# js0n-lai/my-nope-nerf

Measured on AMD Instinct MI355X. Metric: training rays/sec at 1024 rays×128 samples; PSNR parity (±0.1 dB) vs ref, higher is better.
Workload: dtype f32 (f16x3 emulation); 1 GPU; config 2: V_KITTI scene-1 shape 188x621, 1024 rays x 128 samples per GPU, poses fixed, full train_step (render fwd+bwd, rgb-l2+depth-l1, Adam); global_batch=1024, seq_len=128, hidden_dim=256, parallelism=dp1

## Files before the change

my-nope-nerf_amd/csrc/field_bwd.cpp:

```cpp
#include "common.hpp"

#include <cstdlib>
#include <vector>

namespace {

constexpr int L = NERF_BWD_LAYERS;
constexpr int D = 256, HR = 128;
constexpr int OUT_P[L] = {D, D, D, D, D, D, D, D, D, HR};
constexpr int K1[L] = {64, D, D, D, D, D, D, D, D, D};
constexpr int KP[L] = {64, D, D, D, D + 64, D, D, D, D, D + 64};
constexpr int SEG[L] = {0, 0, 0, 0, 1, 0, 0, 0, 0, 2};
constexpr int NREF[L] = {D, D, D, D, D, D, D, D, D, HR};
constexpr int KREF[L] = {63, D, D, D, D + 63, D, D, D, D, D + 27};
constexpr int LF = 8, LR = 9;

struct Carve {
    char* base;
    size_t off = 0;
    float* take(size_t n) {
        off = (off + 255) & ~size_t(255);
        float* p = base ? reinterpret_cast<float*>(base + off) : nullptr;
        off += n * sizeof(float);
        return p;
    }
};

struct Work {
    float *graw4, *dyr, *dyr_rm, *dyr_cm, *part, *hpart, *scratch;
    float *dx[L], *dx_rm[L], *dx_cm[L];
    float *genc_p0, *genc_p4, *genc_d;
    float *slab[L], *bslab[L];
    int splits[L];
};

size_t carve(char* base, int np, int ray_grad, Work& w) {
    Carve c{base};
    w.graw4 = c.take((size_t)np * 4);
    w.dyr = c.take((size_t)np * HR);
    w.dyr_rm = c.take(np);
    w.dyr_cm = c.take((size_t)(np / 128) * HR);
    w.part = c.take((size_t)nerf_heads_part_size(D, np));
    w.hpart = c.take((size_t)nerf::heads_part_blocks(np) * (256 + 384 + 4));
    w.scratch = c.take(512);
    for (int l = 1; l < L; ++l) {
        w.dx[l] = c.take((size_t)np * K1[l]);
        w.dx_rm[l] = c.take(np);
        w.dx_cm[l] = c.take((size_t)(np / 128) * K1[l]);
    }
    w.dx[0] = w.dx_rm[0] = w.dx_cm[0] = nullptr;
    w.genc_p0 = ray_grad ? c.take((size_t)np * 64) : nullptr;
    w.genc_p4 = ray_grad ? c.take((size_t)np * 64) : nullptr;
    w.genc_d = ray_grad ? c.take((size_t)np * 64) : nullptr;
    for (int l = 0; l < L; ++l) w.splits[l] = nerf_linear_bwd_weight_splits(OUT_P[l], K1[l], np);
    for (int l = 0; l < L; ++l) {
        w.slab[l] = c.take((size_t)w.splits[l] * OUT_P[l] * KP[l]);
        w.bslab[l] = c.take((size_t)w.splits[l] * OUT_P[l]);
    }
    return c.off + 256;
}

struct EventPool {
    std::vector<hipEvent_t> ev;
    size_t next = 0;
    hipEvent_t get() {
        if (next == ev.size()) {
            hipEvent_t e;
            if (hipEventCreateWithFlags(&e, hipEventDisableTiming) != hipSuccess) return nullptr;
            ev.push_back(e);
        }
        return ev[next++];
    }
};
thread_local EventPool g_events;

#define RC(x)                \
    do {                     \
        const int rc_ = (x); \
        if (rc_) return rc_; \
    } while (0)

int fork(hipStream_t main, hipStream_t side) {
    hipEvent_t e = g_events.get();
    NERF_CHECK(e != nullptr, "nerf_field_backward: hipEventCreate failed");
    NERF_CHECK(hipEventRecord(e, main) == hipSuccess && hipStreamWaitEvent(side, e, 0) == hipSuccess,
// ... 23 lines not shown
    hipStream_t main = nerf::as_stream(stream), side = nerf::as_stream(side_stream);
    nerf_chain_bwd c{};
    c.graw4 = graw4;
    c.hr_mask = a.mask[LR];
    c.ld_hr_mask = HR / 32;
    c.wd = a.wd;
    c.wc = a.wc;
    for (int i = 0; i < 9; ++i) {
        const int l = LR - i;
        c.wt_img[i] = a.wt_cimg[l];
        c.wt_img_rows[i] = KP[l];
        c.in_mask[i] = l == LR ? nullptr : a.mask[l - 1];
        c.ld_in_mask[i] = OUT_P[l - 1 < 0 ? 0 : l - 1] / 32;
    }
    c.dy[0] = w.dyr; c.lddy[0] = HR; c.dy_cmax[0] = w.dyr_cm; c.dy_rmax[0] = w.dyr_rm;
    for (int i = 1; i < 10; ++i) {
        const int l = 10 - i;
        c.dy[i] = w.dx[l]; c.lddy[i] = K1[l]; c.dy_cmax[i] = w.dx_cm[l]; c.dy_rmax[i] = w.dx_rm[l];
    }
    c.scratch = w.scratch;
    c.n_pad = np;
    RC(nerf_mlp_chain_bwd(&c, stream));
    if (heads_after) {
        RC(nerf_heads_bwd_mode(2, graw4, a.act[7], D, a.act[LR], HR, nullptr, 0, D, a.wc, nullptr, 0, w.part, np,
                               nullptr, nullptr, stream));
        RC(nerf_heads_reduce(w.part, D, np, a.g_wd, a.g_bd, a.g_wc, a.g_bc, 0, stream));
    }
    auto dy_of = [&](int l, const float*& dy, const float*& cm, const float*& rm) {
        if (l == LR) { dy = w.dyr; cm = w.dyr_cm; rm = w.dyr_rm; }
        else { dy = w.dx[l + 1]; cm = w.dx_cm[l + 1]; rm = w.dx_rm[l + 1]; }
    };
    const char* ws = std::getenv("NERF_WGRAD_SCHED");
    const int sched = ws ? std::atoi(ws) : 3;
    if (sched == 3) {
        nerf::SlabJobDesc jobs[nerf::kSlabJobsMax];
        int nj = 0;
        for (int e = 0; e < n_extra; ++e) jobs[nj++] = extra[e];
        auto flush = [&](hipStream_t s) -> int {
            if (s != main) RC(fork(main, s));
            RC(nerf::slab_reduce_jobs(jobs, nj, s));
            nj = 0;
            return NERF_OK;
        };
        auto job = [&](int l) {
            jobs[nj++] = nerf::SlabJobDesc{w.slab[l], w.splits[l], OUT_P[l], KP[l], NREF[l], KREF[l], w.bslab[l], a.gw[l],
                                           a.gb[l]};
        };
        auto enc_rows = [&](int l) -> int {
            if (!a.ray_grad) return NERF_OK;
            const float *dy, *cm, *rm;
            dy_of(l, dy, cm, rm);
            const int op = OUT_P[l];
            const int k0 = l == 0 ? 0 : K1[l];
            float* out = l == LR ? w.genc_d : l == 4 ? w.genc_p4 : w.genc_p0;
            return nerf_linear_bwd_data(dy, op, op, a.wt[l] + (size_t)k0 * op, a.wt_img[l] + (size_t)k0 * 8, KP[l], nullptr,
                                        0, nullptr, nullptr, 0, out, 64, np, 64, rm, nullptr, nullptr, stream);
        };
        nerf_wgrad_tile_job tj[nerf::kWgradJobsMax];
        int tgrp[nerf::kWgradJobsMax];
        int nt = 0, cur_grp = 0;
        auto tiles = [&](int l) {
            const float *dy, *cm, *rm;
            dy_of(l, dy, cm, rm);
            const int op = OUT_P[l];
            const float* x = l == 0 ? a.enc_p : a.act[l - 1];
            const float* xcm = l == 0 ? a.enc_p_cmax : a.cmax[l - 1];
            tgrp[nt] = cur_grp;
            tj[nt++] = nerf_wgrad_tile_job{dy, op, op, x, K1[l], K1[l], w.splits[l], w.slab[l], KP[l], 0, w.bslab[l], cm, xcm};
            if (SEG[l]) {
                tgrp[nt] = cur_grp;
                tj[nt++] = nerf_wgrad_tile_job{dy, op, op, SEG[l] == 1 ? a.enc_p : a.enc_d, 64, 64, w.splits[l], w.slab[l],
                                               KP[l], K1[l], nullptr, cm, SEG[l] == 1 ? a.enc_p_cmax : a.enc_d_cmax};
            }
            job(l);
        };
        auto launch = [&]() -> int {
            RC(nerf_linear_bwd_weight_jobs(tj, nt, np, w.splits[LF], stream));
            nt = 0;
            return NERF_OK;
        };
        const char* wgg = std::getenv("NERF_WGRAD_GROUPS");
        const int groups = w.splits[LF] % 16 == 0 ? (wgg ? std::atoi(wgg) : 2) : 0;
        const int s2 = w.splits[LF] / 2;
        if (groups >= 2) {
            for (int l : {LF, 7, 6, 5}) w.splits[l] = s2;
            w.splits[LR] = 2 * s2;
            tiles(LR);
            tgrp[nt - 1] = 1;
            for (int l : {LF, 7}) tiles(l);
            cur_grp = 1;
            for (int l : {6, 5}) tiles(l);
            cur_grp = 0;
            RC(nerf_linear_bwd_weight_job_groups(tj, tgrp, nt, np, s2, 2, stream));
            nt = 0;
        } else {
            for (int l : {LR, LF, 7, 6, 5}) tiles(l);
            RC(launch());
        }
        const char* b1 = std::getenv("NERF_WGRAD_BATCH1");
        const int batch1 = b1 ? std::atoi(b1) : 2;
        if (batch1 != 2) RC(flush(batch1 == 0 ? side : main));
        RC(enc_rows(LR));
        if (groups >= 1) {
            for (int l : {1, 2, 3, 4}) w.splits[l] = s2;
            w.splits[0] = 2 * s2;
            tiles(4);
            tgrp[nt - 1] = 1;
            for (int l : {3, 0}) tiles(l);
            cur_grp = 1;
            for (int l : {2, 1}) tiles(l);
            cur_grp = 0;
            RC(nerf_linear_bwd_weight_job_groups(tj, tgrp, nt, np, s2, 2, stream));
            nt = 0;
        } else {
            for (int l : {3, 2, 1, 4, 0}) tiles(l);
            RC(launch());
        }
        RC(flush(main));
        RC(enc_rows(4));
        RC(enc_rows(0));
    } else if (sched == 2) {
        nerf::SlabJobDesc jobs[nerf::kSlabJobsMax];
        int nj = 0;
        for (int e = 0; e < n_extra; ++e) jobs[nj++] = extra[e];
        auto flush = [&](hipStream_t s) -> int {
            if (s != main) RC(fork(main, s));
            RC(nerf::slab_reduce_jobs(jobs, nj, s));
            nj = 0;
            return NERF_OK;
        };
        auto job = [&](int l) {
            jobs[nj++] = nerf::SlabJobDesc{w.slab[l], w.splits[l], OUT_P[l], KP[l], NREF[l], KREF[l], w.bslab[l], a.gw[l],
                                           a.gb[l]};
        };
        auto enc_rows = [&](int l) -> int {
            if (!a.ray_grad) return NERF_OK;
            const float *dy, *cm, *rm;
            dy_of(l, dy, cm, rm);
            const int op = OUT_P[l];
            const int k0 = l == 0 ? 0 : K1[l];
            float* out = l == LR ? w.genc_d : l == 4 ? w.genc_p4 : w.genc_p0;
            return nerf_linear_bwd_data(dy, op, op, a.wt[l] + (size_t)k0 * op, a.wt_img[l] + (size_t)k0 * 8, KP[l], nullptr,
                                        0, nullptr, nullptr, 0, out, 64, np, 64, rm, nullptr, nullptr, stream);
        };
        {
            const float *dy, *cm, *rm;
            dy_of(LR, dy, cm, rm);
            RC(nerf_linear_bwd_weight(dy, HR, HR, a.act[LF], K1[LR], K1[LR], np, w.splits[LR], w.slab[LR], KP[LR], 0,
                                      w.bslab[LR], cm, a.cmax[LF], stream));
            RC(nerf_linear_bwd_weight(dy, HR, HR, a.enc_d, 64, 64, np, w.splits[LR], w.slab[LR], KP[LR], K1[LR], nullptr,
                                      cm, a.enc_d_cmax, stream));
            job(LR);
            RC(enc_rows(LR));
        }
        {
            nerf_wgrad_job wj[nerf::kWgradPairsMax];
            int n = 0;
            for (int l = LF; l >= 1; --l) {
                const float *dy, *cm, *rm;
                dy_of(l, dy, cm, rm);
                NERF_CHECK(OUT_P[l] == D && K1[l] == D && w.splits[l] == w.splits[LF], "layer %d", l);
                wj[n++] = nerf_wgrad_job{dy, D, a.act[l - 1], D, w.slab[l], KP[l], w.bslab[l], cm, a.cmax[l - 1]};
                if (l != 4) job(l);
            }
            RC(nerf_linear_bwd_weight_multi(wj, n, np, w.splits[LF], stream));
        }
        RC(flush(side));
        {
            const float *dy4, *cm4, *rm4, *dy0, *cm0, *rm0;
            dy_of(4, dy4, cm4, rm4);
            dy_of(0, dy0, cm0, rm0);
            RC(nerf::wgrad_narrow_pair(dy4, D, a.enc_p, 64, w.splits[4], w.slab[4], KP[4], K1[4], nullptr, cm4, a.enc_p_cmax,
                                       dy0, D, a.enc_p, 64, w.splits[0], w.slab[0], KP[0], 0, w.bslab[0], cm0, a.enc_p_cmax,
                                       np, main));
            job(4);
            job(0);
            RC(enc_rows(4));
            RC(enc_rows(0));
        }
        RC(flush(main));
    } else {
        nerf::SlabJobDesc jobs[nerf::kSlabJobsMax];
        int nj = 0;
        for (int e = 0; e < n_extra; ++e) jobs[nj++] = extra[e];
        auto flush = [&](hipStream_t s) -> int {
            if (s != main) RC(fork(main, s));
            RC(nerf::slab_reduce_jobs(jobs, nj, s));
            nj = 0;
            return NERF_OK;
        };
// ... 278 lines not shown
```

my-nope-nerf_amd/csrc/gemm.hpp:

```cpp
#pragma once
#include "common.hpp"

namespace nerf {

typedef float f32x16 __attribute__((ext_vector_type(16)));

__device__ __forceinline__ int acc_row(int r, int hi) { return (r & 3) + 8 * (r >> 2) + 4 * hi; }

template <int TM, int TN>
__device__ __forceinline__ void zero_acc(f32x16 (&acc)[TM][TN]) {
#pragma unroll
    for (int i = 0; i < TM; ++i)
#pragma unroll
        for (int j = 0; j < TN; ++j)
#pragma unroll
            for (int r = 0; r < 16; ++r) acc[i][j][r] = 0.f;
}

struct NTArgs {
    const float* a1; int lda1; int k1;
    const float* a2; int lda2; int k2;
    const float* b;  int ldb;
    const uint16_t* bs; int bs_rows;
    const float* bias;
// ... 456 lines not shown
            }
        }
    }
    if (HD && nh) {
#pragma unroll
        for (int i = 0; i < TM; ++i)
#pragma unroll
            for (int c = 0; c < 3; ++c)
                if (c < nh) {
                    const float v = hp[c][i] + __shfl_xor(hp[c][i], 32, 64);
                    if (hf == 0) lhs[(wm0 + 32 * i + sl) * 3 + c] = v;
                }
    }
    if constexpr (H) {
#pragma unroll
        for (int i = 0; i < TM; ++i) {
            const float m = fmaxf(rmx[i], __shfl_xor(rmx[i], 32, 64));
            if (hf == 0) atomicMax(lrm + wm0 + 32 * i + sl, __float_as_uint(m));
        }
        if (lcm) {
            int base = 0;
            bfly_max_dpp<NV / 2, 8>(cmx, sl, base);
            bfly_max_dpp<NV / 4, 4>(cmx, sl, base);
            bfly_max_dpp<NV / 8, 2>(cmx, sl, base);
            bfly_max_dpp<NV / 16, 1>(cmx, sl, base);
            bfly_max<NV / 32, 16>(cmx, sl, base);
            constexpr int n = NV / 32 > 1 ? NV / 32 : 1;
            uint32_t* g = lcm + (wm0 / 128) * lcm_ld;
#pragma unroll
            for (int t = 0; t < n; ++t) {
                const int f = base + t;
                atomicMax(g + wn0 + 32 * (f >> 4) + 4 * hf + 8 * ((f >> 2) & 3) + (f & 3), __float_as_uint(cmx[t]));
            }
        }
    }
}

template <int TM, int TN, bool H = false>
__device__ __forceinline__ void tn_store_lds(const TNArgs& p, f32x16 (&acc)[TM][TN], char* smem, int split, int o0,
                                             int j0, int wm0, int wn0, const int* lea = nullptr,
                                             const int* leb = nullptr) {
    using T = TileLds<TN>;
    if (p.ablate & 1) {
        tn_store(p, acc, split, o0, j0, wm0, wn0);
        return;
    }
    float* slab = p.slab + (size_t)split * p.slab_stride;
    float* wlds = reinterpret_cast<float*>(smem + (threadIdx.x >> 6) * T::BYTES);
    write_tile_lds<TM, TN>(acc, wlds, [&](int rl, int c4, float4 v) {
        if constexpr (H) {
            const int ea = lea[wm0 + rl];
            const int4 eb = *reinterpret_cast<const int4*>(leb + wn0 + c4);
            v.x = __builtin_amdgcn_ldexpf(v.x, -(ea + eb.x));
            v.y = __builtin_amdgcn_ldexpf(v.y, -(ea + eb.y));
            v.z = __builtin_amdgcn_ldexpf(v.z, -(ea + eb.z));
            v.w = __builtin_amdgcn_ldexpf(v.w, -(ea + eb.w));
        }
        float* d = slab + (size_t)(o0 + wm0 + rl) * p.ldslab + p.col0 + j0 + wn0 + c4;
        {
            store_out4(d, v);
        }
    });
}

inline int tn_xcd_group(int policy, int nout, int kin, int splits) {
    return (policy >= 7 && nout == 256 && kin == 256 && splits % 8 == 0) ? 2 : 0;
}

int dispatch_nt_x6(const NTArgs& a, int epi, int policy, hipStream_t s, double flops, bool h16 = false);
int dispatch_tn_x6(const TNArgs& a, int nout, int kin, int splits, int policy, hipStream_t s, double flops,
                   bool h16 = false);
bool tn_seg_supported(int nout, int k1, int k2, int splits);
int dispatch_tn_x6_seg(const TNArgs& pm, const TNArgs& ps, int nout, int splits, int policy, hipStream_t s,
                       double flops);
bool wgrad_supported(int nout, int kin, int splits, int rows_per_split);
bool wgrad_seg_supported(int nout, int k1, int k2, int splits, int rows_per_split);
void launch_wgrad(const TNArgs& a, int nout, int kin, int splits, hipStream_t s);
void launch_wgrad_seg(const TNArgs& pm, const TNArgs& ps, int nout, int splits, hipStream_t s);
struct TNPairs {
    TNArgs a[kWgradPairsMax];
    int n;
};
void launch_wgrad_pairs(const TNPairs& m, int splits, hipStream_t s);
enum WgradJobKind : int { WJ_PAIR = 0, WJ_WIDE = 1, WJ_ENC = 2, WJ_ENC_HALF = 3, WJ_ENC128 = 4 };
struct TNJobs {
    TNArgs a[kWgradJobsMax];
    int kind[kWgradJobsMax];
    int grp[kWgradJobsMax];
    int n;
    int ngroups;
};
void launch_wgrad_jobs(const TNJobs& m, int splits, hipStream_t s);
void launch_wgrad_two(const TNArgs& a, int na, const TNArgs& b, int nb, hipStream_t s);

}
```

my-nope-nerf_amd/csrc/gemm_f32.hip:

```cpp
#include "gemm.hpp"

#include <cstdlib>

namespace nerf {

constexpr int BK = 32;

template <int TM, int TN, int LDA, int LDB, bool SWAP = false>
__device__ __forceinline__ void mfma_tile(const float* __restrict__ As, const float* __restrict__ Bs,
                                          int wm0, int wn0, f32x16 (&acc)[TM][TN]) {
    const int lane = lane_id();
    const int l32 = lane & 31;
    const int hi = lane >> 5;
    float a0[TM], b0[TN], a1[TM], b1[TN];
    auto rd = [&](int kp, float (&ra)[TM], float (&rb)[TN]) {
        const int k = 2 * kp + hi;
#pragma unroll
        for (int i = 0; i < TM; ++i) ra[i] = As[k * LDA + wm0 + 32 * i + l32];
#pragma unroll
        for (int j = 0; j < TN; ++j) rb[j] = Bs[k * LDB + wn0 + 32 * j + l32];
    };
    auto mm = [&](const float (&ra)[TM], const float (&rb)[TN]) {
#pragma unroll
        for (int i = 0; i < TM; ++i)
// ... 441 lines not shown
    a.cm_groups = (dy_cmax && x_cmax && m % 128 == 0) ? m / 128 : 0;
    a.stamps = g_stamps;
    return NERF_OK;
}

extern "C" int nerf_linear_bwd_weight(const float* dy, int lddy, int nout, const float* x, int ldx,
                                      int kin, int m, int splits, float* slab, int ldslab, int col0,
                                      float* bslab, const float* dy_cmax, const float* x_cmax, void* stream) {
    TNArgs a;
    int rc = tn_args(__func__, dy, lddy, nout, x, ldx, kin, m, splits, slab, ldslab, col0, bslab, dy_cmax, x_cmax, a);
    if (rc) return rc;
    const bool h16 = g_precision == 2 && dy_cmax && x_cmax && (m / splits) % 128 == 0;
    hipStream_t s = as_stream(stream);
    const double fl = 2.0 * m * nout * (double)kin;
    prof_next(nout % 256 == 0 && kin % 256 == 0 ? NERF_PROF_DW : NERF_PROF_DW_NARROW,
              4.0 * m * (double)(nout + kin) + 4.0 * nout * (double)kin + (bslab ? 4.0 * nout : 0.0));
    const int pol = g_tn_policy ? g_tn_policy : kTnDefault;
    if (g_precision >= 1) return dispatch_tn_x6(a, nout, kin, splits, pol, s, fl, h16);
    prof_begin(s);
    if (pol >= 3 && nout % 256 == 0 && kin % 256 == 0) {
        dim3 grid(nout / 256, kin / 256, splits);
        hipLaunchKernelGGL((k_gemm_tn<256, 256, 2, 4>), grid, dim3(512), 0, s, a);
    } else if (nout % 128 == 0 && kin % 128 == 0) {
        dim3 grid(nout / 128, kin / 128, splits);
        hipLaunchKernelGGL((k_gemm_tn<128, 128, 2, 2>), grid, dim3(256), 0, s, a);
    } else if (nout % 128 == 0) {
        dim3 grid(nout / 128, kin / 64, splits);
        hipLaunchKernelGGL((k_gemm_tn<128, 64, 4, 1>), grid, dim3(256), 0, s, a);
    } else if (kin % 128 == 0) {
        dim3 grid(nout / 64, kin / 128, splits);
        hipLaunchKernelGGL((k_gemm_tn<64, 128, 2, 2>), grid, dim3(256), 0, s, a);
    } else {
        dim3 grid(nout / 64, kin / 64, splits);
        hipLaunchKernelGGL((k_gemm_tn<64, 64, 2, 2>), grid, dim3(256), 0, s, a);
    }
    prof_end(s, fl, 1);
    return check_launch(__func__);
}

extern "C" int nerf_linear_bwd_weight_multi(const nerf_wgrad_job* j, int n, int m, int splits, void* stream) {
    NERF_CHECK_PTR(j);
    hipStream_t s = as_stream(stream);
    NERF_CHECK(n >= 1 && n <= kWgradPairsMax, "%s: %d layers (1..%d)", __func__, n, kWgradPairsMax);
    const int pol = g_tn_policy ? g_tn_policy : kTnDefault;
    bool fused = n > 1 && g_precision == 2 && pol == 8 && splits > 0 && m % splits == 0 && (m / splits) % 128 == 0 &&
                 wgrad_supported(256, 256, splits, m / splits);
    TNPairs tp{};
    for (int i = 0; i < n && fused; ++i) {
        fused = j[i].dy_cmax && j[i].x_cmax;
        int rc = tn_args(__func__, j[i].dy, j[i].lddy, 256, j[i].x, j[i].ldx, 256, m, splits, j[i].slab, j[i].ldslab, 0,
                         j[i].bslab, j[i].dy_cmax, j[i].x_cmax, tp.a[i]);
        if (rc) return rc;
    }
    if (!fused) {
        for (int i = 0; i < n; ++i) {
            int rc = nerf_linear_bwd_weight(j[i].dy, j[i].lddy, 256, j[i].x, j[i].ldx, 256, m, splits, j[i].slab,
                                            j[i].ldslab, 0, j[i].bslab, j[i].dy_cmax, j[i].x_cmax, s);
            if (rc) return rc;
        }
        return NERF_OK;
    }
    tp.n = n;
    prof_next(NERF_PROF_DW, n * (4.0 * m * 512.0 + 4.0 * 256 * 256 + 4.0 * 256));
    prof_begin(s);
    launch_wgrad_pairs(tp, splits, s);
    prof_end(s, n * 2.0 * m * 256.0 * 256.0, 3);
    return check_launch("k_wgrad_pairs");
}

extern "C" int nerf_linear_bwd_weight_job_groups(const nerf_wgrad_tile_job* j, const int* group, int n, int m,
                                                 int splits, int n_groups, void* stream) {
    NERF_CHECK_PTR(j);
    hipStream_t s = as_stream(stream);
    NERF_CHECK(n >= 1 && n <= kWgradJobsMax, "%s: %d jobs (1..%d)", __func__, n, kWgradJobsMax);
    NERF_CHECK(n_groups >= 1 && n_groups <= 4, "%s: n_groups %d (1..4)", __func__, n_groups);
    for (int i = 0; i < n; ++i)
        NERF_CHECK(group == nullptr ? n_groups == 1 : (group[i] >= 0 && group[i] < n_groups),
                   "%s: job %d: group %d of %d", __func__, i, group ? group[i] : 0, n_groups);
    const int pol = g_tn_policy ? g_tn_policy : kTnDefault;
    bool fused = g_precision == 2 && pol == 8 && splits > 0 && splits % 8 == 0;
    TNJobs tj{};
    tj.ngroups = n_groups;
    double bytes = 0.0, flops = 0.0;
    for (int i = 0; i < n && fused; ++i) {
        const nerf_wgrad_tile_job& q = j[i];
        const bool twice = q.splits == 2 * splits, once = q.splits == splits;
        int kind = -1;
        if (q.nout == 256 && q.kin == 256 && once) kind = WJ_PAIR;
        else if (q.nout == 128 && q.kin == 256 && twice) kind = WJ_WIDE;
        else if (q.nout == 256 && q.kin == 64 && twice) kind = WJ_ENC;
        else if (q.nout == 256 && q.kin == 64 && once) kind = WJ_ENC_HALF;
        else if (q.nout == 128 && q.kin == 64 && twice) kind = WJ_ENC128;
        fused = kind >= 0 && q.dy_cmax && q.x_cmax && m % q.splits == 0 && (m / q.splits) % 128 == 0 &&
                wgrad_supported(q.nout, q.kin, q.splits, m / q.splits);
        if (!fused) break;
        int rc = tn_args(__func__, q.dy, q.lddy, q.nout, q.x, q.ldx, q.kin, m, q.splits, q.slab, q.ldslab, q.col0,
                         q.bslab, q.dy_cmax, q.x_cmax, tj.a[i]);
        if (rc) return rc;
        tj.kind[i] = kind;
        tj.grp[i] = group ? group[i] : 0;
        bytes += 4.0 * m * (q.kin + (q.col0 == 0 ? q.nout : 0)) + 4.0 * q.nout * q.kin + (q.bslab ? 4.0 * q.nout : 0.0);
        flops += 2.0 * m * q.nout * q.kin;
    }
    if (!fused) {
        for (int i = 0; i < n; ++i) {
            const nerf_wgrad_tile_job& q = j[i];
            int rc = nerf_linear_bwd_weight(q.dy, q.lddy, q.nout, q.x, q.ldx, q.kin, m, q.splits, q.slab, q.ldslab,
                                            q.col0, q.bslab, q.dy_cmax, q.x_cmax, s);
            if (rc) return rc;
        }
        return NERF_OK;
    }
    tj.n = n;
    prof_next(NERF_PROF_DW, bytes);
    prof_begin(s);
    launch_wgrad_jobs(tj, splits, s);
    prof_end(s, flops, 3);
    return check_launch("k_wgrad_jobs");
}

extern "C" int nerf_linear_bwd_weight_jobs(const nerf_wgrad_tile_job* j, int n, int m, int splits, void* stream) {
    return nerf_linear_bwd_weight_job_groups(j, nullptr, n, m, splits, 1, stream);
}

namespace nerf {
int wgrad_narrow_pair(const float* dy_a, int lddy_a, const float* x_a, int ldx_a, int splits_a, float* slab_a,
                      int ldslab_a, int col0_a, float* bslab_a, const float* dcm_a, const float* xcm_a,
                      const float* dy_b, int lddy_b, const float* x_b, int ldx_b, int splits_b, float* slab_b,
                      int ldslab_b, int col0_b, float* bslab_b, const float* dcm_b, const float* xcm_b, int m,
                      hipStream_t s) {
    const int pol = g_tn_policy ? g_tn_policy : kTnDefault;
    const bool fused = g_precision == 2 && pol == 8 && dcm_a && xcm_a && dcm_b && xcm_b && m % splits_a == 0 &&
                       m % splits_b == 0 && (m / splits_a) % 128 == 0 && (m / splits_b) % 128 == 0 &&
                       wgrad_supported(256, 64, splits_a, m / splits_a) && wgrad_supported(256, 64, splits_b, m / splits_b);
    if (!fused) {
        int rc = nerf_linear_bwd_weight(dy_a, lddy_a, 256, x_a, ldx_a, 64, m, splits_a, slab_a, ldslab_a, col0_a, bslab_a,
                                        dcm_a, xcm_a, s);
        if (rc) return rc;
        return nerf_linear_bwd_weight(dy_b, lddy_b, 256, x_b, ldx_b, 64, m, splits_b, slab_b, ldslab_b, col0_b, bslab_b,
                                      dcm_b, xcm_b, s);
    }
    TNArgs a, b;
    int rc = tn_args(__func__, dy_a, lddy_a, 256, x_a, ldx_a, 64, m, splits_a, slab_a, ldslab_a, col0_a, bslab_a, dcm_a,
                     xcm_a, a);
    if (rc) return rc;
    rc = tn_args(__func__, dy_b, lddy_b, 256, x_b, ldx_b, 64, m, splits_b, slab_b, ldslab_b, col0_b, bslab_b, dcm_b, xcm_b,
                 b);
    if (rc) return rc;
    prof_next(NERF_PROF_DW_NARROW, 2 * (4.0 * m * 320.0 + 4.0 * 256 * 64) + (bslab_a ? 1024.0 : 0.0) + (bslab_b ? 1024.0 : 0.0));
    prof_begin(s);
    launch_wgrad_two(a, splits_a, b, splits_b, s);
    prof_end(s, 2 * 2.0 * m * 256.0 * 64.0, 3);
    return check_launch("k_wgrad_two");
}
}

extern "C" int nerf_linear_bwd_weight_seg(const float* dy, int lddy, int nout, const float* x1, int ldx1, int k1,
                                          const float* x2, int ldx2, int k2, int m, int splits, float* slab,
                                          int ldslab, float* bslab, const float* dy_cmax, const float* x1_cmax,
                                          const float* x2_cmax, void* stream) {
    TNArgs pm, ps;
    int rc = tn_args(__func__, dy, lddy, nout, x1, ldx1, k1, m, splits, slab, ldslab, 0, bslab, dy_cmax, x1_cmax, pm);
    if (rc) return rc;
    rc = tn_args(__func__, dy, lddy, nout, x2, ldx2, k2, m, splits, slab, ldslab, k1, nullptr, dy_cmax, x2_cmax, ps);
    if (rc) return rc;
    const int pol = g_tn_policy ? g_tn_policy : kTnDefault;
    const bool one = g_precision == 2 && pol >= 7 && dy_cmax && x1_cmax && x2_cmax && (m / splits) % 128 == 0 &&
                     tn_seg_supported(nout, k1, k2, splits);
    if (!one) {
        rc = nerf_linear_bwd_weight(dy, lddy, nout, x1, ldx1, k1, m, splits, slab, ldslab, 0, bslab, dy_cmax, x1_cmax,
                                    stream);
        if (rc) return rc;
        return nerf_linear_bwd_weight(dy, lddy, nout, x2, ldx2, k2, m, splits, slab, ldslab, k1, nullptr, dy_cmax,
                                      x2_cmax, stream);
    }
    const double fl = 2.0 * m * nout * (double)(k1 + k2);
    prof_next(nout % 256 == 0 ? NERF_PROF_DW : NERF_PROF_DW_NARROW,
              4.0 * m * (double)(nout + k1 + k2) + 4.0 * nout * (double)(k1 + k2) + (bslab ? 4.0 * nout : 0.0));
    return dispatch_tn_x6_seg(pm, ps, nout, splits, pol, as_stream(stream), fl);
}

static int slab_job_check(const char* fn, const SlabJob& j) {
    NERF_CHECK(j.slab && j.gw, "%s: null slab / gradient", fn);
    NERF_CHECK(j.splits > 0 && j.nout > 0 && j.kin_ref > 0 && j.ldslab >= j.kin_ref && j.nout_ref <= j.nout &&
                   j.nout_ref > 0,
               "%s: bad sizes", fn);
    return NERF_OK;
}
static int slab_job_blocks(const SlabJob& j) {
    const int cblocks = (j.kin_ref + SR_COLS - 1) / SR_COLS;
    const int bias_blocks = (j.bslab && j.gb) ? (j.nout_ref + SR_COLS - 1) / SR_COLS : 0;
    return j.nout_ref * cblocks + bias_blocks;
}

extern "C" int nerf_slab_reduce(const float* slab, int splits, int nout, int ldslab, int nout_ref,
                                int kin_ref, const float* bslab, float* gw, float* gb, int accumulate,
// ... 69 lines not shown
```

my-nope-nerf_amd/csrc/wgrad.hip:

```cpp
#include "gemm.hpp"
#include "x16.hpp"

#include <utility>

namespace nerf {
namespace wg {

constexpr int NTH = 512;
constexpr int KS = 32;
constexpr int NS = 3;

template <int BO, int BK>
struct Cfg {
    static constexpr int CA = BO / 64, CB = BK / 64;
    static constexpr int WO = BO / 2, WK = BK / 2;
    static constexpr int TM = WO / 32, TN = WK / 32;
    static constexpr int AH = BO * 16 + 128, BH = BK * 16 + 128;
    static constexpr int AP = 2 * AH, BP = 2 * BH;
    static constexpr int KSTEP = 2 * AP + 2 * BP;
    static constexpr int BUF = 2 * KSTEP;
    static constexpr int LOOP = 2 * BUF;
    static constexpr int EPI = 4 * TileLds<TN>::BYTES;
    static constexpr int MAIN = LOOP > EPI ? LOOP : EPI;
    static constexpr int BYTES = MAIN + 2 * (BO + BK) * 4 + 4 * BO * 4;
// ... 118 lines not shown
        auto iter = [&](int s, auto uc) {
            put(uc, smem + ((s + 1) & 1) * C::BUF, s + 1 < nst);
            load(uc, s + 1 + NS);
            if constexpr (BIAS) {
                if (s == nst - 1) {
#pragma unroll
                    for (int c = 0; c < CA; ++c) lbias[lw * BO + CA * lane + c] = bsum[c];
                }
            }
            __syncthreads();
        };
        int s = 0;
        for (; s + NS <= nst; s += NS)
            unroll<NS>([&](auto r) {
                constexpr int R = decltype(r)::value;
                iter(s + R, std::integral_constant<int, (R + 1) % NS>{});
            });
        unroll<NS - 1>([&](auto r) {
            constexpr int R = decltype(r)::value;
            if (s + R < nst) iter(s + R, std::integral_constant<int, (R + 1) % NS>{});
        });
    } else {
        exponents();
        const int l32 = lane & 31, hi = lane >> 5;
        const int wm0 = (wave >> 1) * C::WO, wn0 = (wave & 1) * C::WK;
        f32x16 acc[TM][TN];
        zero_acc(acc);
        uint4 fa[2][TM][2], fb[2][TN][2];
        auto frag = [&](auto kc, const char* ks) {
            constexpr int K = decltype(kc)::value;
#pragma unroll
            for (int j = 0; j < TN; ++j)
#pragma unroll
                for (int q = 0; q < 2; ++q)
                    fb[K][j][q] = *reinterpret_cast<const uint4*>(ks + 2 * C::AP + q * C::BP + hi * C::BH + swz(wn0 + 32 * j + l32) * 16);
#pragma unroll
            for (int i = 0; i < TM; ++i)
#pragma unroll
                for (int q = 0; q < 2; ++q)
                    fa[K][i][q] = *reinterpret_cast<const uint4*>(ks + q * C::AP + hi * C::AH + swz(wm0 + 32 * i + l32) * 16);
        };
        auto mma = [&](auto kc) {
            constexpr int K = decltype(kc)::value;
#pragma unroll
            for (int i = 0; i < TM; ++i)
#pragma unroll
                for (int j = 0; j < TN; ++j) {
                    f32x16 c = acc[i][j];
                    c = mfma_f16(fa[K][i][0], fb[K][j][1], c);
                    c = mfma_f16(fa[K][i][1], fb[K][j][0], c);
                    c = mfma_f16(fa[K][i][0], fb[K][j][0], c);
                    acc[i][j] = c;
                }
        };
        constexpr std::integral_constant<int, 0> k0{};
        constexpr std::integral_constant<int, 1> k1{};
        __syncthreads();
        frag(k0, smem);
        for (int s = 0; s < nst; ++s) {
            const char* cur = smem + (s & 1) * C::BUF;
            frag(k1, cur + C::KSTEP);
            __builtin_amdgcn_sched_barrier(0);
            mma(k0);
            __syncthreads();
            frag(k0, smem + ((s + 1) & 1) * C::BUF);
            __builtin_amdgcn_sched_barrier(0);
            mma(k1);
        }
        if constexpr (BIAS) {
            for (int c = tid; c < BO; c += NTH / 2)
                p.bslab[(size_t)split * p.nout + o0 + c] =
                    ((lbias[c] + lbias[BO + c]) + lbias[2 * BO + c]) + lbias[3 * BO + c];
        }
        tn_store_lds<TM, TN, true>(p, acc, smem, split, o0, j0, wm0, wn0, lea, leb);
    }
}

template <int BO, int BK, int AUX = Cfg<BO, BK>::MAIN, int SET = BO + BK, int NS = wg::NS>
__device__ __forceinline__ void block_any(const TNArgs& p, char* smem, int o0, int jt, int split, int par = 0) {
    if (jt == 0 && p.bslab != nullptr) block<BO, BK, true, AUX, SET, NS>(p, smem, o0, jt, split, par);
    else block<BO, BK, false, AUX, SET, NS>(p, smem, o0, jt, split, par);
}

constexpr int cmax(int a, int b) { return a > b ? a : b; }
constexpr int JOBS_AUX = cmax(cmax(Cfg<256, 128>::MAIN, Cfg<128, 256>::MAIN), cmax(Cfg<256, 64>::MAIN, Cfg<128, 64>::MAIN));
constexpr int JOBS_SET = cmax(cmax(256 + 128, 128 + 256), cmax(256 + 64, 128 + 64));
constexpr int JOBS_BYTES = JOBS_AUX + 2 * JOBS_SET * 4 + 4 * 256 * 4;
static_assert(JOBS_SET == 384, "exponent sets");

}

__global__ __launch_bounds__(wg::NTH, 2) void k_wgrad_pair(TNArgs p) {
    __shared__ __attribute__((aligned(16))) char smem[wg::Cfg<256, 128>::BYTES];
    const int w = blockIdx.x, slot = w >> 3;
    wg::block_any<256, 128>(p, smem, 0, slot & 1, (slot >> 1) * 8 + (w & 7));
}

__global__ __launch_bounds__(wg::NTH, 2) void k_wgrad_pairs(TNPairs m) {
    __shared__ __attribute__((aligned(16))) char smem[wg::Cfg<256, 128>::BYTES];
    const int w = blockIdx.x, slot = w >> 3;
    for (int i = 0; i < m.n; ++i)
        wg::block_any<256, 128>(m.a[i], smem, 0, slot & 1, (slot >> 1) * 8 + (w & 7), i & 1);
}

template <int SH>
__global__ __launch_bounds__(wg::NTH, 2) void k_wgrad_jobs(TNJobs m) {
    __shared__ __attribute__((aligned(16))) char smem[wg::JOBS_BYTES];
    constexpr int A = wg::JOBS_AUX;
    constexpr int NSJ = SH == 3 ? 4 : wg::NS;
    const int per = gridDim.x / m.ngroups;
    const int gsel = blockIdx.x / per;
    const int w = blockIdx.x - gsel * per, q = w >> 3;
    const int jt = q & 1, sp = (q >> 1) * 8 + (w & 7);
    int c = 0;
    auto pairs = [&]() {
        for (int i = 0; i < m.n; ++i)
            if (m.kind[i] == WJ_PAIR && m.grp[i] == gsel)
                wg::block_any<256, 128, A, wg::JOBS_SET, NSJ>(m.a[i], smem, 0, jt, sp, c++ & 1);
    };
    auto narrow = [&]() {
        for (int i = 0; i < m.n; ++i) {
            const int k = m.kind[i];
            if ((k == WJ_ENC128 || k == WJ_ENC_HALF) && m.grp[i] == gsel)
                wg::block_any<128, 64, A, wg::JOBS_SET, NSJ>(m.a[i], smem, k == WJ_ENC_HALF ? 128 * jt : 0, 0,
                                          k == WJ_ENC_HALF ? sp : 2 * sp + jt, c++ & 1);
        }
    };
    if constexpr (SH & 1) {
        for (int i = 0; i < m.n; ++i)
            if (m.kind[i] == WJ_WIDE && m.grp[i] == gsel)
                wg::block_any<128, 256, A, wg::JOBS_SET, NSJ>(m.a[i], smem, 0, 0, 2 * sp + jt, c++ & 1);
        if constexpr (SH & 2) narrow();
        pairs();
    } else if (m.ngroups > 1) {
        if constexpr (SH & 2) narrow();
        pairs();
    } else {
        pairs();
        if constexpr (SH & 2) narrow();
    }
    if constexpr (SH & 4)
        for (int i = 0; i < m.n; ++i)
            if (m.kind[i] == WJ_ENC && m.grp[i] == gsel)
                wg::block_any<256, 64, A, wg::JOBS_SET, NSJ>(m.a[i], smem, 0, 0, 2 * sp + jt, c++ & 1);
}

__global__ __launch_bounds__(wg::NTH, 2) void k_wgrad_two(TNArgs a, int na, TNArgs b) {
    __shared__ __attribute__((aligned(16))) char smem[wg::Cfg<256, 64>::BYTES];
    const int w = blockIdx.x;
    if (w < na) wg::block_any<256, 64>(a, smem, 0, 0, w);
    else wg::block_any<256, 64>(b, smem, 0, 0, w - na);
}

template <int BO, int BK>
__global__ __launch_bounds__(wg::NTH, 2) void k_wgrad_one(TNArgs p) {
    __shared__ __attribute__((aligned(16))) char smem[wg::Cfg<BO, BK>::BYTES];
    wg::block_any<BO, BK>(p, smem, 0, 0, blockIdx.x);
}

template <int BO, int BK, int CT, int BK2>
__global__ __launch_bounds__(wg::NTH, 2) void k_wgrad_seg(TNArgs pm, TNArgs ps) {
    constexpr int B1 = wg::Cfg<BO, BK>::BYTES, B2 = wg::Cfg<BO, BK2>::BYTES;
    __shared__ __attribute__((aligned(16))) char smem[B1 > B2 ? B1 : B2];
    const int w = blockIdx.x, slot = w >> 3;
    const int jt = slot % (CT + 1), split = (slot / (CT + 1)) * 8 + (w & 7);
    if (jt < CT) wg::block_any<BO, BK>(pm, smem, 0, jt, split);
    else wg::block_any<BO, BK2>(ps, smem, 0, 0, split);
}

bool wgrad_supported(int nout, int kin, int splits, int rows_per_split) {
    if (rows_per_split % wg::KS != 0 || rows_per_split < 3 * wg::KS) return false;
    return (nout == 256 && kin == 256 && splits % 8 == 0) || (nout == 256 && kin == 64) ||
           (nout == 128 && (kin == 256 || kin == 64));
}
bool wgrad_seg_supported(int nout, int k1, int k2, int splits, int rows_per_split) {
    return rows_per_split % wg::KS == 0 && rows_per_split >= 3 * wg::KS && k1 == 256 && k2 == 64 &&
           (nout == 256 || nout == 128) && splits % 8 == 0;
}

void launch_wgrad(const TNArgs& a, int nout, int kin, int splits, hipStream_t s) {
    if (nout == 256 && kin == 256)
        hipLaunchKernelGGL(k_wgrad_pair, dim3(2 * splits), dim3(wg::NTH), 0, s, a);
    else if (nout == 256)
        hipLaunchKernelGGL((k_wgrad_one<256, 64>), dim3(splits), dim3(wg::NTH), 0, s, a);
    else if (kin == 256)
        hipLaunchKernelGGL((k_wgrad_one<128, 256>), dim3(splits), dim3(wg::NTH), 0, s, a);
    else
        hipLaunchKernelGGL((k_wgrad_one<128, 64>), dim3(splits), dim3(wg::NTH), 0, s, a);
}

void launch_wgrad_two(const TNArgs& a, int na, const TNArgs& b, int nb, hipStream_t s) {
    hipLaunchKernelGGL(k_wgrad_two, dim3(na + nb), dim3(wg::NTH), 0, s, a, na, b);
}

void launch_wgrad_pairs(const TNPairs& m, int splits, hipStream_t s) {
    hipLaunchKernelGGL(k_wgrad_pairs, dim3(2 * splits), dim3(wg::NTH), 0, s, m);
}

void launch_wgrad_jobs(const TNJobs& m, int splits, hipStream_t s) {
    int sh = 0;
    for (int i = 0; i < m.n; ++i)
        sh |= m.kind[i] == WJ_WIDE ? 1 : m.kind[i] == WJ_ENC128 || m.kind[i] == WJ_ENC_HALF ? 2 : m.kind[i] == WJ_ENC ? 4 : 0;
    const dim3 g(2 * splits * m.ngroups), b(wg::NTH);
    switch (sh) {
    case 0: hipLaunchKernelGGL(k_wgrad_jobs<0>, g, b, 0, s, m); break;
    case 1: hipLaunchKernelGGL(k_wgrad_jobs<1>, g, b, 0, s, m); break;
    case 2: hipLaunchKernelGGL(k_wgrad_jobs<2>, g, b, 0, s, m); break;
    case 3: hipLaunchKernelGGL(k_wgrad_jobs<3>, g, b, 0, s, m); break;
    case 4: hipLaunchKernelGGL(k_wgrad_jobs<4>, g, b, 0, s, m); break;
    case 5: hipLaunchKernelGGL(k_wgrad_jobs<5>, g, b, 0, s, m); break;
    case 6: hipLaunchKernelGGL(k_wgrad_jobs<6>, g, b, 0, s, m); break;
    default: hipLaunchKernelGGL(k_wgrad_jobs<7>, g, b, 0, s, m); break;
    }
}

void launch_wgrad_seg(const TNArgs& pm, const TNArgs& ps, int nout, int splits, hipStream_t s) {
    if (nout == 256)
        hipLaunchKernelGGL((k_wgrad_seg<256, 128, 2, 64>), dim3(3 * splits), dim3(wg::NTH), 0, s, pm, ps);
    else
        hipLaunchKernelGGL((k_wgrad_seg<128, 256, 1, 64>), dim3(2 * splits), dim3(wg::NTH), 0, s, pm, ps);
}

}
```

Measured before the change: 571,200 rays/s.

## Fuse skip-segment weight-grad tiles and rebalance layer groups in wgrad job launches

Adds a fused segmented weight-gradient block that computes the main 256-column input and the 64-column encoding skip input in one tile, sharing the dy loads and MFMA A fragments. Adjacent main/encoding job pairs are detected at launch time and rewritten to the new fused kinds when a matching kernel specialization exists. A new default schedule (NERF_WGRAD_FUSE=1) redistributes layers across the two launch groups so the encoding-carrying layers sit next to each other. The aim is to cut redundant dy loads, per-job LDS staging and tail imbalance between groups. In exchange the larger exponent set raises LDS use, and the kernel adds template variants.

```diff
diff --git a/my-nope-nerf_amd/csrc/field_bwd.cpp b/my-nope-nerf_amd/csrc/field_bwd.cpp
--- a/my-nope-nerf_amd/csrc/field_bwd.cpp
+++ b/my-nope-nerf_amd/csrc/field_bwd.cpp
@@ -1,6 +1,7 @@
 #include "common.hpp"
 
 #include <cstdlib>
+#include <initializer_list>
 #include <vector>
 
 namespace {
@@ -190,11 +191,26 @@
         const char* wgg = std::getenv("NERF_WGRAD_GROUPS");
         const int groups = w.splits[LF] % 16 == 0 ? (wgg ? std::atoi(wgg) : 2) : 0;
         const int s2 = w.splits[LF] / 2;
-        if (groups >= 2) {
+        const char* wfu = std::getenv("NERF_WGRAD_FUSE");
+        const int fuse = groups >= 2 ? (wfu ? std::atoi(wfu) : 1) : 0;
+        auto deal = [&](std::initializer_list<int> g0, std::initializer_list<int> g1) -> int {
+            for (int l : g0) tiles(l);
+            cur_grp = 1;
+            for (int l : g1) tiles(l);
+            cur_grp = 0;
+            RC(nerf_linear_bwd_weight_job_groups(tj, tgrp, nt, np, s2, 2, stream));
+            nt = 0;
+            return NERF_OK;
+        };
+        if (fuse == 1) {
+            for (int l : {LF, 7, 6, 5, 4, 3, 2, 1}) w.splits[l] = s2;
+            w.splits[LR] = w.splits[0] = 2 * s2;
+            RC(deal({7, 6}, {4, LF}));
+        } else if (groups >= 2) {
             for (int l : {LF, 7, 6, 5}) w.splits[l] = s2;
             w.splits[LR] = 2 * s2;
             tiles(LR);
-            tgrp[nt - 1] = 1;
+            if (fuse == 0) tgrp[nt - 1] = 1;
             for (int l : {LF, 7}) tiles(l);
             cur_grp = 1;
             for (int l : {6, 5}) tiles(l);
@@ -209,11 +225,13 @@
         const int batch1 = b1 ? std::atoi(b1) : 2;
         if (batch1 != 2) RC(flush(batch1 == 0 ? side : main));
         RC(enc_rows(LR));
-        if (groups >= 1) {
+        if (fuse == 1) {
+            RC(deal({5, 3, 0}, {LR, 2, 1}));
+        } else if (groups >= 1) {
             for (int l : {1, 2, 3, 4}) w.splits[l] = s2;
             w.splits[0] = 2 * s2;
             tiles(4);
-            tgrp[nt - 1] = 1;
+            if (fuse == 0) tgrp[nt - 1] = 1;
             for (int l : {3, 0}) tiles(l);
             cur_grp = 1;
             for (int l : {2, 1}) tiles(l);
diff --git a/my-nope-nerf_amd/csrc/gemm.hpp b/my-nope-nerf_amd/csrc/gemm.hpp
--- a/my-nope-nerf_amd/csrc/gemm.hpp
+++ b/my-nope-nerf_amd/csrc/gemm.hpp
@@ -562,7 +562,8 @@
     int n;
 };
 void launch_wgrad_pairs(const TNPairs& m, int splits, hipStream_t s);
-enum WgradJobKind : int { WJ_PAIR = 0, WJ_WIDE = 1, WJ_ENC = 2, WJ_ENC_HALF = 3, WJ_ENC128 = 4 };
+enum WgradJobKind : int { WJ_PAIR = 0, WJ_WIDE = 1, WJ_ENC = 2, WJ_ENC_HALF = 3, WJ_ENC128 = 4, WJ_SEG256 = 5, WJ_SEG128 = 6,
+                          WJ_SEG2 = 7 };
 struct TNJobs {
     TNArgs a[kWgradJobsMax];
     int kind[kWgradJobsMax];
@@ -571,6 +572,7 @@
     int ngroups;
 };
 void launch_wgrad_jobs(const TNJobs& m, int splits, hipStream_t s);
+bool wgrad_jobs_shapes_compiled(int sh);
 void launch_wgrad_two(const TNArgs& a, int na, const TNArgs& b, int nb, hipStream_t s);
 
 }
diff --git a/my-nope-nerf_amd/csrc/gemm_f32.hip b/my-nope-nerf_amd/csrc/gemm_f32.hip
--- a/my-nope-nerf_amd/csrc/gemm_f32.hip
+++ b/my-nope-nerf_amd/csrc/gemm_f32.hip
@@ -547,6 +547,7 @@
     TNJobs tj{};
     tj.ngroups = n_groups;
     double bytes = 0.0, flops = 0.0;
+    int sh = 0;
     for (int i = 0; i < n && fused; ++i) {
         const nerf_wgrad_tile_job& q = j[i];
         const bool twice = q.splits == 2 * splits, once = q.splits == splits;
@@ -564,6 +565,7 @@
         if (rc) return rc;
         tj.kind[i] = kind;
         tj.grp[i] = group ? group[i] : 0;
+        sh |= kind == WJ_WIDE ? 1 : kind == WJ_ENC128 || kind == WJ_ENC_HALF ? 2 : kind == WJ_ENC ? 4 : 0;
         bytes += 4.0 * m * (q.kin + (q.col0 == 0 ? q.nout : 0)) + 4.0 * q.nout * q.kin + (q.bslab ? 4.0 * q.nout : 0.0);
         flops += 2.0 * m * q.nout * q.kin;
     }
@@ -577,6 +579,28 @@
         return NERF_OK;
     }
     tj.n = n;
+    {
+        int kind[kWgradJobsMax], shf = 0;
+        for (int i = 0; i < n; ++i) kind[i] = tj.kind[i];
+        for (int i = 0; i + 1 < n; ++i) {
+            const nerf_wgrad_tile_job &p = j[i], &q = j[i + 1];
+            const bool l4 = kind[i] == WJ_PAIR && kind[i + 1] == WJ_ENC_HALF;
+            const bool colour = kind[i] == WJ_WIDE && kind[i + 1] == WJ_ENC128;
+            if ((l4 || colour) && p.kin == 256 && p.col0 == 0 && q.kin == 64 && q.col0 == p.kin && q.bslab == nullptr &&
+                q.dy == p.dy && q.lddy == p.lddy && q.nout == p.nout && q.dy_cmax == p.dy_cmax && q.splits == p.splits &&
+                q.slab == p.slab && q.ldslab == p.ldslab && tj.grp[i] == tj.grp[i + 1]) {
+                kind[i] = l4 ? WJ_SEG256 : WJ_SEG128;
+                kind[i + 1] = WJ_SEG2;
+                ++i;
+            }
+        }
+        for (int i = 0; i < n; ++i) {
+            const int k = kind[i];
+            shf |= k == WJ_WIDE ? 1 : k == WJ_ENC128 || k == WJ_ENC_HALF ? 2 : k == WJ_ENC ? 4 : k == WJ_SEG256 ? 8 : k == WJ_SEG128 ? 16 : 0;
+        }
+        if (shf != sh && wgrad_jobs_shapes_compiled(shf))
+            for (int i = 0; i < n; ++i) tj.kind[i] = kind[i];
+    }
     prof_next(NERF_PROF_DW, bytes);
     prof_begin(s);
     launch_wgrad_jobs(tj, splits, s);
diff --git a/my-nope-nerf_amd/csrc/wgrad.hip b/my-nope-nerf_amd/csrc/wgrad.hip
--- a/my-nope-nerf_amd/csrc/wgrad.hip
+++ b/my-nope-nerf_amd/csrc/wgrad.hip
@@ -224,11 +224,246 @@
     else block<BO, BK, false, AUX, SET, NS>(p, smem, o0, jt, split, par);
 }
 
+template <int BO, int BK, int BE>
+struct CfgSeg {
+    static constexpr int BT = BK + BE;
+    static constexpr int CA = BO / 64, CB = BK / 64;
+    static constexpr int GN = BK / 128, GM = 4 / GN;
+    static constexpr int TM = 2, TN = 5;
+    static constexpr int EN = BE / 8;
+    static constexpr int AH = BO * 16 + 128, BH = BT * 16 + 128;
+    static constexpr int AP = 2 * AH, BP = 2 * BH;
+    static constexpr int KSTEP = 2 * AP + 2 * BP;
+    static constexpr int BUF = 2 * KSTEP;
+    static constexpr int LOOP = 2 * BUF;
+    static constexpr int EPI = 4 * TileLds<2>::BYTES;
+    static constexpr int MAIN = LOOP > EPI ? LOOP : EPI;
+    static_assert(BO == 64 * GM && BK == 128 * GN && BE == 32 * GN && (GN == 1 || GN == 2), "fused tile");
+};
+
+template <int J0, int NJ, int TM, int TN, typename Emit>
+__device__ __forceinline__ void write_tile_cols(f32x16 (&acc)[TM][TN], float* wlds, Emit&& emit) {
+    f32x16 sub[TM][NJ];
+#pragma unroll
+    for (int i = 0; i < TM; ++i)
+#pragma unroll
+        for (int j = 0; j < NJ; ++j) sub[i][j] = acc[i][J0 + j];
+    write_tile_lds<TM, NJ>(sub, wlds, emit);
+}
+
+template <int BO, int BK, int BE, bool BIAS, int AUX, int SET, int NS>
+__device__ __forceinline__ void block_seg(const TNArgs& pm, const TNArgs& ps, char* smem, int jt, int split, int par) {
+    using C = CfgSeg<BO, BK, BE>;
+    constexpr int CA = C::CA, CB = C::CB, TM = C::TM, TN = C::TN, EN = C::EN;
+    int tid = threadIdx.x;
+    asm volatile("" : "+v"(tid));
+    const int lane = tid & 63;
+    const int wave = __builtin_amdgcn_readfirstlane(tid >> 6);
+    const int j0 = jt * BK, e0 = jt * BE;
+    const size_t s0 = (size_t)split * pm.rows_per_split;
+    const int nst = pm.rows_per_split / KS;
+    static_assert(AUX >= C::MAIN, "aux region");
+    static_assert(SET >= BO + C::BT, "an exponent set holds BO + BK + BE ints");
+    int* lea = reinterpret_cast<int*>(smem + AUX) + par * SET;
+    int* leb = lea + BO;
+    float* lbias = reinterpret_cast<float*>(smem + AUX) + 2 * SET;
+    auto exponents = [&]() {
+        for (int e = tid; e < BO; e += NTH) lea[e] = row_exp(tn_colmax(pm.cm_dy, pm.ldcm_dy, s0, pm.rows_per_split, e));
+        for (int e = tid; e < BK; e += NTH) leb[e] = row_exp(tn_colmax(pm.cm_x, pm.ldcm_x, s0, pm.rows_per_split, j0 + e));
+        for (int e = tid; e < BE; e += NTH)
+            leb[BK + e] = row_exp(tn_colmax(ps.cm_x, ps.ldcm_x, s0, pm.rows_per_split, e0 + e));
+        __syncthreads();
+    };
+
+    if (wave >= 4) {
+        const int lw = wave - 4;
+        const __amdgpu_buffer_rsrc_t rdy = __builtin_amdgcn_make_buffer_rsrc(
+            (void*)(pm.dy + s0 * pm.lddy), (short)0, pm.rows_per_split * pm.lddy * 4, 0x00020000);
+        const __amdgpu_buffer_rsrc_t rx = __builtin_amdgcn_make_buffer_rsrc(
+            (void*)(pm.x + s0 * pm.ldx + j0), (short)0, (pm.rows_per_split * pm.ldx - j0) * 4, 0x00020000);
+        const __amdgpu_buffer_rsrc_t re = __builtin_amdgcn_make_buffer_rsrc(
+            (void*)(ps.x + s0 * ps.ldx + e0), (short)0, (pm.rows_per_split * ps.ldx - e0) * 4, 0x00020000);
+        int va_off = 4 * CA * lane, vb_off = 4 * CB * lane;
+        const int ecol = BE == 64 ? lane : lane >> 1, eh = BE == 64 ? 0 : lane & 1;
+        int ve_off = (4 * eh * ps.ldx + ecol) * 4;
+        float va[NS][8][CA], vb[NS][8][CB], ve[NS][EN];
+        auto load = [&](auto uc, int t) {
+            constexpr int U = decltype(uc)::value;
+            t = t < nst ? t : nst - 1;
+            const int r0 = KS * t + 8 * lw;
+#pragma unroll
+            for (int i = 0; i < 8; ++i) {
+                load_row<CA>(va[U][i], rdy, va_off, (r0 + i) * pm.lddy * 4);
+                load_row<CB>(vb[U][i], rx, vb_off, (r0 + i) * pm.ldx * 4);
+            }
+#pragma unroll
+            for (int i = 0; i < EN; ++i) {
+                float t1[1];
+                load_row<1>(t1, re, ve_off, (r0 + i) * ps.ldx * 4);
+                ve[U][i] = t1[0];
+            }
+        };
+        unroll<NS>([&](auto u) { load(u, decltype(u)::value); });
+        exponents();
+        int ea[CA], eb[CB];
+#pragma unroll
+        for (int c = 0; c < CA; ++c) ea[c] = lea[CA * lane + c];
+#pragma unroll
+        for (int c = 0; c < CB; ++c) eb[c] = leb[CB * lane + c];
+        const int ee = leb[BK + ecol];
+        float bsum[CA];
+#pragma unroll
+        for (int c = 0; c < CA; ++c) bsum[c] = 0.f;
+        auto put = [&](auto uc, char* buf, bool real) {
+            constexpr int U = decltype(uc)::value;
+            char* ks = buf + (lw >> 1) * C::KSTEP;
+#pragma unroll
+            for (int c = 0; c < CA; ++c) {
+                __builtin_amdgcn_sched_barrier(0);
+                float v[8];
+#pragma unroll
+                for (int i = 0; i < 8; ++i) v[i] = va[U][i][c];
+                put_strip(ks + (lw & 1) * C::AH + swz(CA * lane + c) * 16, C::AP, v, ea[c]);
+                if constexpr (BIAS) {
+                    float sm = 0.f;
+#pragma unroll
+                    for (int i = 0; i < 8; ++i) sm += v[i];
+                    bsum[c] += real ? sm : 0.f;
+                }
+            }
+#pragma unroll
+            for (int c = 0; c < CB; ++c) {
+                __builtin_amdgcn_sched_barrier(0);
+                float v[8];
+#pragma unroll
+                for (int i = 0; i < 8; ++i) v[i] = vb[U][i][c];
+                put_strip(ks + 2 * C::AP + (lw & 1) * C::BH + swz(CB * lane + c) * 16, C::BP, v, eb[c]);
+            }
+            __builtin_amdgcn_sched_barrier(0);
+            char* de = ks + 2 * C::AP + (lw & 1) * C::BH + swz(BK + ecol) * 16;
+            if constexpr (BE == 64) {
+                float v[8];
+#pragma unroll
+                for (int i = 0; i < 8; ++i) v[i] = ve[U][i];
+                put_strip(de, C::BP, v, ee);
+            } else {
+                uint32_t h[2], l[2];
+                split2h(ve[U][0], ve[U][1], ee, h[0], l[0]);
+                split2h(ve[U][2], ve[U][3], ee, h[1], l[1]);
+                *reinterpret_cast<uint2*>(de + 8 * eh) = make_uint2(h[0], h[1]);
+                *reinterpret_cast<uint2*>(de + 8 * eh + C::BP) = make_uint2(l[0], l[1]);
+            }
+            __builtin_amdgcn_sched_barrier(0);
+        };
+        put(std::integral_constant<int, 0>{}, smem, true);
+        asm volatile("" : "+v"(va_off), "+v"(vb_off), "+v"(ve_off));
+        load(std::integral_constant<int, 0>{}, NS);
+        __syncthreads();
+        auto iter = [&](int s, auto uc) {
+            put(uc, smem + ((s + 1) & 1) * C::BUF, s + 1 < nst);
+            load(uc, s + 1 + NS);
+            if constexpr (BIAS) {
+                if (s == nst - 1) {
+#pragma unroll
+                    for (int c = 0; c < CA; ++c) lbias[lw * BO + CA * lane + c] = bsum[c];
+                }
+            }
+            __syncthreads();
+        };
+        int s = 0;
+        for (; s + NS <= nst; s += NS)
+            unroll<NS>([&](auto r) {
+                constexpr int R = decltype(r)::value;
+                iter(s + R, std::integral_constant<int, (R + 1) % NS>{});
+            });
+        unroll<NS - 1>([&](auto r) {
+            constexpr int R = decltype(r)::value;
+            if (s + R < nst) iter(s + R, std::integral_constant<int, (R + 1) % NS>{});
+        });
+    } else {
+        exponents();
+        const int l32 = lane & 31, hi = lane >> 5;
+        const int wq = wave % C::GN;
+        const int wm0 = (wave / C::GN) * 64, wn0 = wq * 128, we0 = BK + wq * 32;
+        f32x16 acc[TM][TN];
+        zero_acc(acc);
+        uint4 fa[TM][2], fb[TN][2];
+        auto frag = [&](const char* ks) {
+#pragma unroll
+            for (int j = 0; j < TN; ++j)
+#pragma unroll
+                for (int q = 0; q < 2; ++q)
+                    fb[j][q] = *reinterpret_cast<const uint4*>(ks + 2 * C::AP + q * C::BP + hi * C::BH +
+                                                               swz((j < 4 ? wn0 + 32 * j : we0) + l32) * 16);
+#pragma unroll
+            for (int i = 0; i < TM; ++i)
+#pragma unroll
+                for (int q = 0; q < 2; ++q)
+                    fa[i][q] = *reinterpret_cast<const uint4*>(ks + q * C::AP + hi * C::AH + swz(wm0 + 32 * i + l32) * 16);
+        };
+        auto mma = [&]() {
+#pragma unroll
+            for (int j = 0; j < TN; ++j)
+#pragma unroll
+                for (int i = 0; i < TM; ++i) {
+                    f32x16 c = acc[i][j];
+                    c = mfma_f16(fa[i][0], fb[j][1], c);
+                    c = mfma_f16(fa[i][1], fb[j][0], c);
+                    c = mfma_f16(fa[i][0], fb[j][0], c);
+                    acc[i][j] = c;
+                }
+        };
+        __syncthreads();
+        for (int s = 0; s < nst; ++s) {
+            const char* cur = smem + (s & 1) * C::BUF;
+            frag(cur);
+            mma();
+            frag(cur + C::KSTEP);
+            mma();
+            __syncthreads();
+        }
+        if constexpr (BIAS) {
+            if (pm.bslab != nullptr)
+                for (int c = tid; c < BO; c += NTH / 2)
+                    pm.bslab[(size_t)split * pm.nout + c] =
+                        ((lbias[c] + lbias[BO + c]) + lbias[2 * BO + c]) + lbias[3 * BO + c];
+        }
+        if (pm.ablate & 1) {
+            tn_store(pm, acc, split, 0, j0, wm0, wn0);
+            return;
+        }
+        float* slab = pm.slab + (size_t)split * pm.slab_stride;
+        float* wlds = reinterpret_cast<float*>(smem + wave * TileLds<2>::BYTES);
+        auto emit_to = [&](int lcol, int scol) {
+            return [&, lcol, scol](int rl, int c4, float4 v) {
+                const int ea = lea[wm0 + rl];
+                const int4 eb = *reinterpret_cast<const int4*>(leb + lcol + c4);
+                v.x = __builtin_amdgcn_ldexpf(v.x, -(ea + eb.x));
+                v.y = __builtin_amdgcn_ldexpf(v.y, -(ea + eb.y));
+                v.z = __builtin_amdgcn_ldexpf(v.z, -(ea + eb.z));
+                v.w = __builtin_amdgcn_ldexpf(v.w, -(ea + eb.w));
+                store_out4(slab + (size_t)(wm0 + rl) * pm.ldslab + scol + c4, v);
+            };
+        };
+        write_tile_cols<0, 2>(acc, wlds, emit_to(wn0, pm.col0 + j0 + wn0));
+        write_tile_cols<2, 2>(acc, wlds, emit_to(wn0 + 64, pm.col0 + j0 + wn0 + 64));
+        write_tile_cols<4, 1>(acc, wlds, emit_to(we0, ps.col0 + e0 + wq * 32));
+    }
+}
+
+template <int BO, int BK, int BE, int AUX, int SET, int NS>
+__device__ __forceinline__ void block_seg_any(const TNArgs& pm, const TNArgs& ps, char* smem, int jt, int split, int par) {
+    if (BK == 256 || (jt == 0 && pm.bslab != nullptr)) block_seg<BO, BK, BE, true, AUX, SET, NS>(pm, ps, smem, jt, split, par);
+    else block_seg<BO, BK, BE, false, AUX, SET, NS>(pm, ps, smem, jt, split, par);
+}
+
 constexpr int cmax(int a, int b) { return a > b ? a : b; }
-constexpr int JOBS_AUX = cmax(cmax(Cfg<256, 128>::MAIN, Cfg<128, 256>::MAIN), cmax(Cfg<256, 64>::MAIN, Cfg<128, 64>::MAIN));
-constexpr int JOBS_SET = cmax(cmax(256 + 128, 128 + 256), cmax(256 + 64, 128 + 64));
+constexpr int JOBS_AUX = cmax(cmax(cmax(Cfg<256, 128>::MAIN, Cfg<128, 256>::MAIN), cmax(Cfg<256, 64>::MAIN, Cfg<128, 64>::MAIN)),
+                              cmax(CfgSeg<256, 128, 32>::MAIN, CfgSeg<128, 256, 64>::MAIN));
+constexpr int JOBS_SET = cmax(cmax(cmax(256 + 128, 128 + 256), cmax(256 + 64, 128 + 64)), cmax(256 + 128 + 32, 128 + 256 + 64));
 constexpr int JOBS_BYTES = JOBS_AUX + 2 * JOBS_SET * 4 + 4 * 256 * 4;
-static_assert(JOBS_SET == 384, "exponent sets");
+static_assert(JOBS_SET == 448, "exponent sets");
+static_assert(JOBS_BYTES <= 160 * 1024, "LDS");
 
 }
 
@@ -268,6 +503,14 @@
                                           k == WJ_ENC_HALF ? sp : 2 * sp + jt, c++ & 1);
         }
     };
+    if constexpr ((SH & 8) != 0)
+        for (int i = 0; i + 1 < m.n; ++i)
+            if (m.kind[i] == WJ_SEG256 && m.grp[i] == gsel)
+                wg::block_seg_any<256, 128, 32, A, wg::JOBS_SET, wg::NS>(m.a[i], m.a[i + 1], smem, jt, sp, c++ & 1);
+    if constexpr ((SH & 16) != 0)
+        for (int i = 0; i + 1 < m.n; ++i)
+            if (m.kind[i] == WJ_SEG128 && m.grp[i] == gsel)
+                wg::block_seg_any<128, 256, 64, A, wg::JOBS_SET, wg::NS>(m.a[i], m.a[i + 1], smem, 0, 2 * sp + jt, c++ & 1);
     if constexpr (SH & 1) {
         for (int i = 0; i < m.n; ++i)
             if (m.kind[i] == WJ_WIDE && m.grp[i] == gsel)
@@ -339,10 +582,14 @@
     hipLaunchKernelGGL(k_wgrad_pairs, dim3(2 * splits), dim3(wg::NTH), 0, s, m);
 }
 
+bool wgrad_jobs_shapes_compiled(int sh) { return sh < 8 || (sh & 3) == 0; }
+
 void launch_wgrad_jobs(const TNJobs& m, int splits, hipStream_t s) {
     int sh = 0;
-    for (int i = 0; i < m.n; ++i)
-        sh |= m.kind[i] == WJ_WIDE ? 1 : m.kind[i] == WJ_ENC128 || m.kind[i] == WJ_ENC_HALF ? 2 : m.kind[i] == WJ_ENC ? 4 : 0;
+    for (int i = 0; i < m.n; ++i) {
+        const int k = m.kind[i];
+        sh |= k == WJ_WIDE ? 1 : k == WJ_ENC128 || k == WJ_ENC_HALF ? 2 : k == WJ_ENC ? 4 : k == WJ_SEG256 ? 8 : k == WJ_SEG128 ? 16 : 0;
+    }
     const dim3 g(2 * splits * m.ngroups), b(wg::NTH);
     switch (sh) {
     case 0: hipLaunchKernelGGL(k_wgrad_jobs<0>, g, b, 0, s, m); break;
@@ -352,7 +599,13 @@
     case 4: hipLaunchKernelGGL(k_wgrad_jobs<4>, g, b, 0, s, m); break;
     case 5: hipLaunchKernelGGL(k_wgrad_jobs<5>, g, b, 0, s, m); break;
     case 6: hipLaunchKernelGGL(k_wgrad_jobs<6>, g, b, 0, s, m); break;
-    default: hipLaunchKernelGGL(k_wgrad_jobs<7>, g, b, 0, s, m); break;
+    case 7: hipLaunchKernelGGL(k_wgrad_jobs<7>, g, b, 0, s, m); break;
+    case 8: hipLaunchKernelGGL(k_wgrad_jobs<8>, g, b, 0, s, m); break;
+    case 12: hipLaunchKernelGGL(k_wgrad_jobs<12>, g, b, 0, s, m); break;
+    case 16: hipLaunchKernelGGL(k_wgrad_jobs<16>, g, b, 0, s, m); break;
+    case 20: hipLaunchKernelGGL(k_wgrad_jobs<20>, g, b, 0, s, m); break;
+    case 24: hipLaunchKernelGGL(k_wgrad_jobs<24>, g, b, 0, s, m); break;
+    default: hipLaunchKernelGGL(k_wgrad_jobs<28>, g, b, 0, s, m); break;
     }
 }
 
```

Result: no change. 576,900 rays/s (median of 6 runs) (+1.0%).
